# cc-ai/climategan

Hardware: AMD Instinct MI355X
Metric: 640x640 images/sec (G+D step): per-domain sample slots per second of the joint Masker+Painter training step (update_G + update_D), global batch 32 per domain (higher is better)
Workload: dtype bf16

## Files before the change

### climategan_amd/_lib.py

```python
import ctypes as C
import os
from pathlib import Path

_HERE = Path(__file__).resolve().parent
LIB_PATH = Path(os.environ["CGAN_LIB"]).resolve() if os.environ.get("CGAN_LIB") else _HERE / "libcgan_hip.so"

CGAN_F16, CGAN_BF16, CGAN_F32 = 0, 1, 2
ACT_NONE, ACT_RELU, ACT_LRELU, ACT_TANH, ACT_SIGMOID = 0, 1, 2, 3, 4
PAD_ZERO, PAD_REFLECT = 0, 1
ABI_VERSION = 1


class ConvDesc(C.Structure):
    _fields_ = [
        ("dtype", C.c_int32), ("n", C.c_int32), ("h_in", C.c_int32), ("w_in", C.c_int32),
        ("c_in", C.c_int32), ("c_out", C.c_int32),
        ("kh", C.c_int32), ("kw", C.c_int32), ("stride", C.c_int32), ("pad", C.c_int32), ("dilation", C.c_int32),
        ("pad_mode", C.c_int32), ("h_out", C.c_int32), ("w_out", C.c_int32), ("in_upsample", C.c_int32),
        ("act", C.c_int32), ("act_slope", C.c_float), ("has_bias", C.c_int32), ("has_residual", C.c_int32),
        ("residual_upsample", C.c_int32),
    ]


class NormStatsDesc(C.Structure):
# ... 121 lines not shown
    "cgan_spade_packed_weight_bytes": (C.c_size_t, [C.POINTER(SpadeDesc)]),
    "cgan_spade_pack_weights": (C.c_int, [_P, _P, _P, _P, _P, _P, _P, C.POINTER(SpadeDesc), _P]),
    "cgan_spade_fused_fwd": (C.c_int, [_P, _P, _P, _P, _P, _P, C.POINTER(SpadeDesc), _P]),
    "cgan_spade_fused_fwd_train": (C.c_int, [_P, _P, _P, _P, _P, _P, _P, C.POINTER(SpadeDesc), _P]),
    "cgan_spectral_norm_workspace_bytes": (C.c_size_t, [C.c_int32, C.c_int32]),
    "cgan_spectral_norm_power_iter": (C.c_int, [_P, _P, _P, _P, C.c_int32, C.c_int32, _P, C.c_size_t, _P]),
    "cgan_spectral_norm_power_iter_batched": (C.c_int, [_P, C.c_int32, C.c_int32, C.c_int32, _P]),
    "cgan_extra_adam_multi_tensor": (C.c_int, [_P, C.c_int32, C.c_int64, C.c_int32, C.c_int32, C.c_int32, C.c_double,
                                               C.c_double, C.c_double, C.c_double, C.c_double, _P]),
    "cgan_grads_nonfinite_check_multi_tensor": (C.c_int, [_P, C.c_int32, C.c_int64, C.c_double, C.c_int32, _P, _P]),
    "cgan_adam_multi_tensor": (C.c_int, [_P, C.c_int32, C.c_int64] + [C.c_double] * 6 + [_P, _P]),
    "cgan_rmsprop_multi_tensor": (C.c_int, [_P, C.c_int32, C.c_int64] + [C.c_double] * 5 + [_P, _P]),
    "cgan_amp_optim_finish": (C.c_int, [_P, C.c_int32, _P, _P]),
    "cgan_nchw_to_nhwc": (C.c_int, [_P, _P, _P, C.c_int32, C.c_int32, C.c_int32, C.c_int32, C.c_int32, C.c_int32, _P]),
    "cgan_nhwc_to_nchw": (C.c_int, [_P, _P, _P, _P, C.c_int32, C.c_int32, C.c_int32, C.c_int32, C.c_int32, C.c_int32, _P]),
    "cgan_resize_nearest_nhwc": (C.c_int, [_P, _P, C.c_int32, C.c_int32, C.c_int32, C.c_int32, C.c_int32, C.c_int32,
                                           C.c_int32, C.c_int32, C.c_int32, _P]),
    "cgan_avgpool3x3s2_nhwc": (C.c_int, [_P, _P, C.c_int32, C.c_int32, C.c_int32, C.c_int32, C.c_int32, _P]),
    "cgan_maxpool3x3s2_nhwc": (C.c_int, [_P, _P, C.c_int32, C.c_int32, C.c_int32, C.c_int32, C.c_int32, _P]),
    "cgan_resize_bilinear_nhwc": (C.c_int, [_P, _P, C.c_int32, C.c_int32, C.c_int32, C.c_int32, C.c_int32, C.c_int32,
                                            C.c_int32, C.c_int32, _P]),
    "cgan_resize_bicubic_nhwc": (C.c_int, [_P, _P, C.c_int32, C.c_int32, C.c_int32, C.c_int32, C.c_int32, C.c_int32,
                                           C.c_int32, _P]),
    "cgan_sumpool2x2_nhwc": (C.c_int, [_P, _P, C.c_int32, C.c_int32, C.c_int32, C.c_int32, C.c_int32, _P]),
    "cgan_reflect_pad_bwd_nhwc": (C.c_int, [_P, _P, C.c_int32, C.c_int32, C.c_int32, C.c_int32, C.c_int32, C.c_int32, _P]),
    "cgan_copy_channels_nhwc": (C.c_int, [_P, _P, C.c_int64, C.c_int32, C.c_int32, C.c_int32, C.c_int32, _P]),
    "cgan_eltwise_nhwc": (C.c_int, [_P, _P, _P, C.c_int32, C.c_int32, C.c_int64, _P]),
    "cgan_fold_bn": (C.c_int, [_P, _P, _P, _P, _P, _P, C.c_float, _P, _P, C.c_int32, C.c_int64, _P]),
    "cgan_act_bwd": (C.c_int, [_P, _P, _P, C.c_int32, C.c_int32, C.c_float, C.c_int64, _P]),
    "cgan_instnorm_act_bwd_workspace_bytes": (C.c_size_t, [C.POINTER(NormStatsDesc)]),
    "cgan_instnorm_act_bwd": (C.c_int, [_P, _P, _P, _P, C.POINTER(NormStatsDesc), C.c_int32, C.c_float, _P, C.c_size_t,
                                        _P]),
    "cgan_spade_bwd_prepare": (C.c_int, [_P, _P, _P, _P, _P, _P, _P, _P, _P, C.POINTER(SpadeDesc), _P]),
    "cgan_spade_hidden_bwd_workspace_bytes": (C.c_size_t, [C.POINTER(SpadeDesc)]),
    "cgan_spade_hidden_bwd": (C.c_int, [_P, _P, _P, _P, _P, _P, _P, _P, C.c_size_t, C.POINTER(SpadeDesc), _P]),
    "cgan_batchnorm_train_stats": (C.c_int, [_P, _P, _P, C.c_float, _P, _P, _P, _P, _P, _P, _P, C.POINTER(NormStatsDesc), _P,
                                             C.c_size_t, _P]),
    "cgan_batchnorm_train_stats_from_partials": (C.c_int, [_P, C.c_int32, _P, _P, C.c_float, _P, _P, _P, _P, _P, _P, _P,
                                                           C.POINTER(NormStatsDesc), _P]),
    "cgan_conv2d_stats_chunk_pixels": (C.c_int32, [C.POINTER(ConvDesc)]),
    "cgan_conv2d_nhwc_fwd_stats": (C.c_int, [_P, _P, _P, _P, _P, C.c_size_t, C.POINTER(ConvDesc), _P]),
    "cgan_bn_train_prepare": (C.c_int, [_P, _P, _P, _P, C.c_float, C.c_float, C.c_int64, _P, _P, _P, _P, _P, C.c_int32, _P]),
    "cgan_batchnorm_act_bwd_workspace_bytes": (C.c_size_t, [C.c_int32]),
    "cgan_batchnorm_act_bwd": (C.c_int, [_P, _P, _P, _P, _P, _P, _P, _P, _P, _P, _P, _P, C.c_int32, C.c_int64, C.c_int32,
                                         C.c_int32, C.c_float, _P, C.c_size_t, _P]),
    "cgan_batchnorm_act_bwd_grouped": (C.c_int, [_P, _P, _P, _P, _P, _P, _P, _P, _P, _P, _P, _P, C.c_int32, C.c_int64,
                                                 C.c_int32, C.c_int32, C.c_int32, C.c_float, _P, C.c_size_t, _P]),
    "cgan_bce_logits_nhwc": (C.c_int, [_P, C.c_int32, C.c_int64, C.c_int32, C.c_float, C.c_float, _P, _P, _P]),
    "cgan_hinge_nhwc": (C.c_int, [_P, C.c_int32, C.c_int64, C.c_int32, C.c_int32, C.c_int32, C.c_float, _P, _P, _P]),
    "cgan_l1_nhwc": (C.c_int, [_P, _P, C.c_int32, C.c_int64, C.c_float, _P, _P, _P]),
    "cgan_mse_const_nhwc": (C.c_int, [_P, C.c_int32, C.c_int64, C.c_int32, C.c_float, C.c_float, _P, _P, _P]),
    "cgan_painter_aux_losses": (C.c_int, [_P, _P, _P, C.c_int32, C.c_int32, C.c_int32, C.c_int32, C.c_float, C.c_float,
                                          C.c_float, C.c_float, _P, _P, _P]),
    "cgan_resize_bicubic_bwd_nhwc": (C.c_int, [_P, _P, C.c_int32, C.c_int32, C.c_int32, C.c_int32, C.c_int32, C.c_int32,
                                               C.c_int32, _P]),
    "cgan_spectral_norm_bwd": (C.c_int, [_P, _P, _P, _P, _P, C.c_int32, C.c_int32, _P, _P]),
    "cgan_painter_heads_fwd": (C.c_int, [_P, _P, _P, _P, _P, C.c_int32, C.c_int32, C.c_int32, C.c_int32, _P]),
    "cgan_painter_heads_bwd": (C.c_int, [_P, _P, _P, _P, C.c_int32, C.c_int32, C.c_int32, C.c_int32, _P]),
    "cgan_diffaug_fwd": (C.c_int, [_P, _P, _P, _P, C.c_int32, C.c_int32, C.c_int32, C.c_int32, C.c_int32, C.c_int32,
                                   C.c_int32, _P, _P]),
    "cgan_diffaug_bwd": (C.c_int, [_P, _P, _P, _P, C.c_int32, C.c_int32, C.c_int32, C.c_int32, C.c_int32, C.c_int32,
                                   C.c_int32, _P, _P]),
    "cgan_painter_heads_diffaug_fwd": (C.c_int, [_P, _P, _P, _P, _P, _P, _P, C.c_int32, C.c_int32, C.c_int32, C.c_int32,
                                                 C.c_int32, C.c_int32, C.c_int32, _P, _P]),
    "cgan_painter_heads_diffaug_bwd": (C.c_int, [_P, _P, _P, _P, _P, _P, C.c_int32, C.c_int32, C.c_int32, C.c_int32,
                                                 C.c_int32, C.c_int32, C.c_int32, _P, _P]),
# ... 142 lines not shown
```

### climategan_amd/autograd.py

```python
import ctypes as C

import os

import torch

from . import ops


GRAD_SCALE = 1.0


def set_grad_scale(s: float):
    global GRAD_SCALE
    GRAD_SCALE = float(s)


BN_GROUPS = 1


class bn_groups:

    def __init__(self, groups: int):
        self.groups = int(groups)

# ... 197 lines not shown
                                       pad_mode=cfg.get("pad_mode", ops.PAD_ZERO), add=add, prepacked=ctx.dgrad,
                                       relu_out=relu_out).t
        dw = db = None
        if ctx.needs_input_grad[1] or (ctx.has_bias and ctx.needs_input_grad[2]):
            dw, db = ops.conv2d_bwd_weight(
                ops.NHWC(x_t, cfg["c_in"]), dy, tuple(weight.shape), stride=cfg["stride"], pad=cfg["pad"],
                dilation=cfg["dilation"], want_bias=ctx.has_bias, pad_mode=cfg.get("pad_mode", ops.PAD_ZERO))
        return dx_t, dw, db, None, None


class InstNormActFn(torch.autograd.Function):

    @staticmethod
    def forward(ctx, x_t, c, eps, act, slope):
        x = ops.NHWC(x_t, c)
        mean, rstd = ops.instnorm_stats(x, eps=eps)
        out = ops.norm_act_apply(x, mean, rstd, act=act, slope=slope)
        ctx.c, ctx.act, ctx.slope = c, act, slope
        ctx.save_for_backward(out.t, rstd)
        return out.t

    @staticmethod
    def backward(ctx, dy_t):
        out_t, rstd = ctx.saved_tensors
        dx = ops.instnorm_act_bwd(ops.NHWC(out_t, ctx.c), ops.NHWC(dy_t.contiguous(), ctx.c), rstd, act=ctx.act,
                                  slope=ctx.slope)
        return dx.t, None, None, None, None


_SPADE_REMAT_GAMMA = os.environ.get("CGAN_SPADE_REMAT_GAMMA") == "1"


_SPADE_FUSED_BWD = os.environ.get("CGAN_SPADE_FUSED_BWD", "1") != "0"


class SpadeFn(torch.autograd.Function):

    @staticmethod
    def forward(ctx, x_t, cond_t, mean, rstd, w_sh, b_sh, w_g, b_g, w_b, b_b, packed, cfg):
        x = ops.NHWC(x_t, cfg["c"])
        cond = ops.NHWC(cond_t, cfg["cond_c"])
        gamma_t = None
        if _SPADE_REMAT_GAMMA or not any(ctx.needs_input_grad):
            y = ops.spade_fused(x, mean, rstd, cond, packed, act=cfg["act"], slope=cfg["slope"],
                                x_upsample=cfg["x_upsample"])
        else:
            y, gamma = ops.spade_fused(x, mean, rstd, cond, packed, act=cfg["act"], slope=cfg["slope"],
                                       x_upsample=cfg["x_upsample"], want_gamma=True)
            gamma_t = gamma.t
        ctx.cfg = cfg
        ctx.save_for_backward(x_t, cond_t, mean, rstd, y.t, w_sh, b_sh, w_g, b_g, w_b, b_b, gamma_t)
        return y.t

    @staticmethod
    def backward(ctx, dy_t):
        cfg = ctx.cfg
        x_t, cond_t, mean, rstd, y_t, w_sh, b_sh, w_g, b_g, w_b, b_b, gamma_t = ctx.saved_tensors
        c, dt = cfg["c"], y_t.dtype
        x, y = ops.NHWC(x_t, c), ops.NHWC(y_t, c)
        dy = ops.NHWC(dy_t.contiguous(), c)
        h, w = y.h, y.w
        seg = ops.resize_nearest(ops.NHWC(cond_t, cfg["cond_c"]), (h, w), cs_out=ops.cs8(cfg["cond_c"]))
        pw_sh = ops.pack_conv_weight(w_sh, b_sh, dt)
        actv = ops.conv2d(seg, pw_sh, pad=1, act=ops.ACT_RELU)
        gamma = ops.NHWC(gamma_t, c) if gamma_t is not None else ops.conv2d(actv, ops.pack_conv_weight(w_g, b_g, dt), pad=1)
        dgb, xhat, dxhat = ops.spade_bwd_prepare(dy, y, x, mean, rstd, gamma, act=cfg["act"], slope=cfg["slope"],
                                                 x_upsample=cfg["x_upsample"])
        del gamma
        w_gb = torch.cat([w_g.detach(), w_b.detach()], dim=0)
        want_gb, want_sh = any(ctx.needs_input_grad[6:10]), any(ctx.needs_input_grad[4:6])
        dw_gb = db_gb = dw_sh = db_sh = None
        if want_gb:
            dw_gb, db_gb = ops.conv2d_bwd_weight(actv, dgb, tuple(w_gb.shape), pad=1)
        fused = (_SPADE_FUSED_BWD and want_sh and not ctx.needs_input_grad[1] and cfg["cond_c"] <= 4 and h * w >= 6400
                 and w_sh.shape[0] == 128 and dgb.t.nbytes < ops.ABI_MAX_BYTES and seg.t.nbytes < ops.ABI_MAX_BYTES)
        d_pre = None
        if fused:
            dw_sh, db_sh = ops.spade_hidden_bwd(dgb, w_gb, seg, pw_sh, c)
        elif want_sh or ctx.needs_input_grad[1]:
            d_pre = ops.conv2d_bwd_data(dgb, w_gb, (actv.n, h, w), pad=1, relu_out=actv)
        del dgb, actv
        if want_sh and not fused:
            dw_sh, db_sh = ops.conv2d_bwd_weight(seg, d_pre, tuple(w_sh.shape), pad=1)
        dcond_t = None
        if ctx.needs_input_grad[1]:
            d_seg = ops.conv2d_bwd_data(d_pre, w_sh.detach(), (seg.n, h, w), pad=1)
            dcond_t = ops.resize_nearest_bwd(d_seg, (cond_t.shape[1], cond_t.shape[2]), cond_t.shape[3]).t
        del d_pre
        if cfg.get("batch_stats"):
            nn_, hh, ww, cs = xhat.t.shape
            dx = ops.instnorm_act_bwd(ops.NHWC(xhat.t.view(1, nn_ * hh * ww, 1, cs), c),
                                      ops.NHWC(dxhat.t.view(1, nn_ * hh * ww, 1, cs), c), rstd[0:1].contiguous(),
                                      act=ops.ACT_NONE)
            dx = ops.NHWC(dx.t.view(nn_, hh, ww, cs), c)
        else:
            dx = ops.instnorm_act_bwd(xhat, dxhat, rstd, act=ops.ACT_NONE)
        if cfg["x_upsample"]:
            dx = ops.sumpool2x2(dx)
        dx_t = dx.t if ctx.needs_input_grad[0] else None
        if not want_gb:
            return (dx_t, dcond_t, None, None, dw_sh, db_sh, None, None, None, None, None, None)
        return (dx_t, dcond_t, None, None, dw_sh, db_sh, dw_gb[:c].contiguous(), db_gb[:c].contiguous(),
                dw_gb[c:].contiguous(), db_gb[c:].contiguous(), None, None)


class MakeMCondFn(torch.autograd.Function):

    @staticmethod
    def forward(ctx, d_t, s_t, x, s_c):
        ctx.s_c, ctx.with_x = s_c, x is not None
        ctx.save_for_backward(d_t, s_t)
        return ops.make_m_cond(ops.NHWC(d_t, 1), ops.NHWC(s_t, s_c), x).t

    @staticmethod
    def backward(ctx, dcond_t):
        d_t, s_t = ctx.saved_tensors
        cond_c = 1 + ctx.s_c + (3 if ctx.with_x else 0)
        dd, ds = ops.make_m_cond_bwd(ops.NHWC(dcond_t.contiguous(), cond_c), ops.NHWC(d_t, 1), ops.NHWC(s_t, ctx.s_c),
                                     ctx.with_x)
        return dd.t, ds.t, None, None


class PainterHeadsFn(torch.autograd.Function):

    @staticmethod
    def forward(ctx, fake_t, x, m, want_d, want_vgg):
        d_in, v_in = ops.painter_heads(ops.NHWC(fake_t, 3), x, m, fake_t.dtype, want_d, want_vgg)
        ctx.save_for_backward(m)
        ctx.want = (want_d, want_vgg)
        empty = fake_t.new_empty(0)
# ... 599 lines not shown
```

### climategan_amd/csrc/train_ops.hip

```cpp
#include "cgan_common.h"

namespace {

__host__ __device__ inline int grid_for_n(long total) {
  long g = (total + 255) / 256;
  return (int)(g < 1 ? 1 : (g > 8192 ? 8192 : g));
}

__device__ __forceinline__ float act_grad_from_out(float out, int act, float slope) {
  switch (act) {
    case CGAN_ACT_RELU: return out > 0.f ? 1.f : 0.f;
    case CGAN_ACT_LRELU: return out > 0.f ? 1.f : slope;
    case CGAN_ACT_TANH: return 1.f - out * out;
    case CGAN_ACT_SIGMOID: return out * (1.f - out);
    default: return 1.f;
  }
}

template <typename T>
__global__ void act_bwd_kernel(const uint16_t* __restrict__ out, const uint16_t* dy, uint16_t* dx, int act, float slope,
                               long groups) {
  for (long i = (long)blockIdx.x * blockDim.x + threadIdx.x; i < groups; i += (long)gridDim.x * blockDim.x) {
    const u32x4 o = CGAN_LD_STREAM(reinterpret_cast<const u32x4*>(out) + i);
    const u32x4 g = CGAN_LD_STREAM(reinterpret_cast<const u32x4*>(dy) + i);
// ... 206 lines not shown
        const float xh = live ? (xv[hh] - mean[(long)n * cs + ch]) * rstd[(long)n * cs + ch] : 0.f;
        rxh[hh] = xh;
        rdx[hh] = dz * (1.f + g2[hh]);
        rdg[hh] = dz * xh;
        dbeta[2 * e + hh] = dz;
      }
      oxh[e] = pack2<T>(rxh[0], rxh[1]);
      odx[e] = pack2<T>(rdx[0], rdx[1]);
      odg[e] = pack2<T>(rdg[0], rdg[1]);
    }
    CGAN_ST_STREAM(oxh, reinterpret_cast<u32x4*>(xhat) + i);
    CGAN_ST_STREAM(odx, reinterpret_cast<u32x4*>(dxhat) + i);
    uint16_t* row = dgb + pix * cs2;
    if (cg * 8 + 8 <= c) {
      *reinterpret_cast<u32x4*>(row + cg * 8) = odg;
    } else {
#pragma unroll
      for (int e = 0; e < 8; ++e)
        if (cg * 8 + e < c) row[cg * 8 + e] = (uint16_t)((odg[e >> 1] >> ((e & 1) * 16)) & 0xffffu);
    }
    if (cg * 8 + 8 <= c && (c & 3) == 0) {
      const u32x4 obt = {pack2<T>(dbeta[0], dbeta[1]), pack2<T>(dbeta[2], dbeta[3]), pack2<T>(dbeta[4], dbeta[5]),
                         pack2<T>(dbeta[6], dbeta[7])};
      if ((c & 7) == 0) {
        *reinterpret_cast<u32x4*>(row + c + cg * 8) = obt;
      } else {
        *reinterpret_cast<u32x2*>(row + c + cg * 8) = (u32x2){obt[0], obt[1]};
        *reinterpret_cast<u32x2*>(row + c + cg * 8 + 4) = (u32x2){obt[2], obt[3]};
      }
    } else {
#pragma unroll
      for (int e = 0; e < 8; ++e)
        if (cg * 8 + e < c) row[c + cg * 8 + e] = bits_of<T>(dbeta[e]);
    }
  }
}

__global__ void bn_train_prepare_kernel(const float* __restrict__ mean, const float* __restrict__ rstd,
                                        const float* __restrict__ gamma, const float* __restrict__ beta, float eps,
                                        float momentum, float count, float* __restrict__ running_mean,
                                        float* __restrict__ running_var, float* __restrict__ mean_out,
                                        float* __restrict__ rstd_out, long long* __restrict__ num_batches_tracked, int c,
                                        int cs) {
  const int ch = blockIdx.x * blockDim.x + threadIdx.x;
  if (ch == 0 && num_batches_tracked) *num_batches_tracked += 1;
  if (ch >= cs) return;
  float m = 0.f, r = 0.f;
  if (ch < c) {
    const float mu = mean[ch], rs = rstd[ch];
    r = rs * (gamma ? gamma[ch] : 1.f);
    m = mu - ((beta && r != 0.f) ? beta[ch] / r : 0.f);
    if (running_mean) {
      const float var_b = 1.f / (rs * rs) - eps;
      const float var_u = count > 1.f ? var_b * count / (count - 1.f) : var_b;
      running_mean[ch] = (1.f - momentum) * running_mean[ch] + momentum * mu;
      running_var[ch] = (1.f - momentum) * running_var[ch] + momentum * var_u;
    }
  }
  mean_out[ch] = m;
  rstd_out[ch] = r;
}

constexpr int BN_BWD_MAX_CHUNKS = 512;
template <int MASK>
__device__ __forceinline__ float bn_bwd_act_grad(float ov, float xv, float fm, float fr, float gneg) {
  if (MASK == 0) return 1.f;
// ... 438 lines not shown
    long blocks = (d->hw + (long)rows * 4 - 1) / ((long)rows * 4);
    const long cap = 8192 / d->n > 0 ? 8192 / d->n : 1;
    blocks = blocks < 1 ? 1 : (blocks > cap ? cap : blocks);
    DISPATCH_T(d->dtype, in_bwd_apply_kernel, dim3((unsigned)blocks, d->n), dim3(256), 0, s, (const uint16_t*)out,
               (const uint16_t*)dy, rstd, (const float*)workspace, (uint16_t*)dx, d->hw, cs, d->c, act, act_slope);
  }
  CGAN_CHECK_LAUNCH("instnorm_act_bwd");
  return CGAN_OK;
}

extern "C" int cgan_spade_bwd_prepare(const void* dy, const void* y, const void* x, const float* mean, const float* rstd,
                                      const void* gamma, void* dgb, void* xhat, void* dxhat, const CganSpadeDesc* d,
                                      void* stream) {
  CGAN_REQUIRE(d && dy && y && x && mean && rstd && gamma && dgb && xhat && dxhat, "spade_bwd_prepare: null pointer");
  CGAN_REQUIRE(d->dtype == CGAN_F16 || d->dtype == CGAN_BF16, "spade_bwd_prepare: bad dtype %d", d->dtype);
  CGAN_REQUIRE(d->n > 0 && d->h > 0 && d->w > 0 && d->c > 0, "spade_bwd_prepare: bad shape");
  CGAN_REQUIRE(d->act == CGAN_ACT_NONE || d->act == CGAN_ACT_LRELU, "spade_bwd_prepare: Unsupported activation: %d", d->act);
  if (d->x_upsample) CGAN_REQUIRE((d->h % 2) == 0 && (d->w % 2) == 0, "spade_bwd_prepare: x_upsample needs even h/w");
  const int cs = cgan_cs(d->c), cs2 = cgan_cs(2 * d->c);
  const long npix = (long)d->n * d->h * d->w;
  hipStream_t s = (hipStream_t)stream;
  if (cs2 != 2 * d->c) {
    hipError_t e = hipMemsetAsync(dgb, 0, (size_t)npix * cs2 * 2, s);
    if (e != hipSuccess) {
      cgan_set_error("spade_bwd_prepare: hipMemsetAsync failed: %s", hipGetErrorString(e));
      return CGAN_ERR_HIP;
    }
  }
  const long groups = npix * (cs / 8);
  DISPATCH_T(d->dtype, spade_bwd_prepare_kernel, dim3(grid_for_n(groups)), dim3(256), 0, s, (const uint16_t*)dy,
             (const uint16_t*)y, (const uint16_t*)x, mean, rstd, (const uint16_t*)gamma, (uint16_t*)dgb, (uint16_t*)xhat,
             (uint16_t*)dxhat, d->h, d->w, d->c, cs, cs2, d->x_upsample, d->act, d->act_slope, groups);
  CGAN_CHECK_LAUNCH("spade_bwd_prepare");
  return CGAN_OK;
}

extern "C" int cgan_bn_train_prepare(const float* batch_mean, const float* batch_rstd, const float* gamma,
                                     const float* beta, float eps, float momentum, int64_t count, float* running_mean,
                                     float* running_var, float* mean_out, float* rstd_out,
                                     int64_t* num_batches_tracked, int32_t c, void* stream) {
  CGAN_REQUIRE(batch_mean && batch_rstd && mean_out && rstd_out, "bn_train_prepare: null pointer");
  CGAN_REQUIRE((running_mean == nullptr) == (running_var == nullptr), "bn_train_prepare: running stats go together");
  CGAN_REQUIRE(c > 0 && count > 0, "bn_train_prepare: bad shape");
  const int cs = cgan_cs(c);
  hipLaunchKernelGGL(bn_train_prepare_kernel, dim3((cs + 255) / 256), dim3(256), 0, (hipStream_t)stream, batch_mean,
                     batch_rstd, gamma, beta, eps, momentum, (float)count, running_mean, running_var, mean_out, rstd_out,
                     (long long*)num_batches_tracked, c, cs);
  CGAN_CHECK_LAUNCH("bn_train_prepare");
  return CGAN_OK;
}

extern "C" size_t cgan_batchnorm_act_bwd_workspace_bytes(int32_t c) {
  return c > 0 ? (size_t)cgan_cs(c) * (3 + 2 * (size_t)BN_BWD_MAX_CHUNKS) * sizeof(float) : 0;
}

extern "C" int cgan_batchnorm_act_bwd(const void* x, const void* out, const void* dy, const float* batch_mean,
                                      const float* batch_rstd, const float* gamma, const float* fold_mean,
                                      const float* fold_rstd, void* dx, float* dgamma, float* dbeta, void* dz_out,
                                      int32_t dtype, int64_t npix, int32_t c, int32_t act, float act_slope,
                                      void* workspace, size_t workspace_bytes, void* stream) {
  return cgan_batchnorm_act_bwd_grouped(x, out, dy, batch_mean, batch_rstd, gamma, fold_mean, fold_rstd, dx, dgamma, dbeta,
                                        dz_out, dtype, npix, c, 1, act, act_slope, workspace, workspace_bytes, stream);
}

extern "C" int cgan_batchnorm_act_bwd_grouped(const void* x, const void* out, const void* dy, const float* batch_mean,
                                              const float* batch_rstd, const float* gamma, const float* fold_mean,
// ... 128 lines not shown
```

### climategan_amd/ops.py

```python
import ctypes as C
import functools
import inspect
import os
from dataclasses import dataclass
from typing import Optional, Tuple

import torch

from . import _lib
from ._lib import (ACT_LRELU, ACT_NONE, ACT_RELU, ACT_SIGMOID, ACT_TANH, CGAN_BF16, CGAN_F16, PAD_REFLECT,
                   PAD_ZERO, ConvDesc, NormStatsDesc, PackItem, SnItem, SpadeDesc)

_DT = {torch.float16: CGAN_F16, torch.bfloat16: CGAN_BF16}


def touch(*tensors) -> None:
    ts = [t for t in tensors if t is not None]
    if ts:
        torch.autograd.graph.increment_version(ts)


MAX_MAP_BYTES = 2 ** 31
ABI_MAX_BYTES = 2 ** 31

# ... 1285 lines not shown
    if x.c != pk.c or cond.c != pk.cond_c:
        raise RuntimeError("spade_fused: channel mismatch (x %d vs %d, cond %d vs %d)" % (x.c, pk.c, cond.c, pk.cond_c))
    if cond.cs != cs4(cond.c):
        raise RuntimeError("spade_fused: cond must be stored with round_up(cond_c,4) channels")
    if x.t.dtype != pk.dtype or cond.t.dtype != pk.dtype:
        raise RuntimeError("spade_fused: dtype mismatch")
    h, w = (x.h * 2, x.w * 2) if x_upsample else (x.h, x.w)
    d = _spade_desc(x.dtype_id, x.n, h, w, x.c, x_upsample, cond.h, cond.w, cond.c, act, slope)
    y = _empty((x.n, h, w, x.cs), dtype=x.t.dtype, device=x.t.device)
    lib = _lib.load()
    if want_gamma:
        gamma = _empty_like(y)
        _lib.check(lib.cgan_spade_fused_fwd_train(_ptr(x.t), _ptr(mean), _ptr(rstd), _ptr(cond.t), _ptr(pk.buf), _ptr(y),
                                                  _ptr(gamma), C.byref(d), _stream()), "cgan_spade_fused_fwd_train")
        return NHWC(y, x.c), NHWC(gamma, x.c)
    _lib.check(lib.cgan_spade_fused_fwd(_ptr(x.t), _ptr(mean), _ptr(rstd), _ptr(cond.t), _ptr(pk.buf), _ptr(y),
                                        C.byref(d), _stream()), "cgan_spade_fused_fwd")
    return NHWC(y, x.c)


@_batch_chunked("dy", "y", "x", "mean", "rstd", "gamma", out_bytes_per_sample=lambda g: g("y").h * g("y").w * cs8(2 * g("y").c) * 2)
def spade_bwd_prepare(dy: NHWC, y: NHWC, x: NHWC, mean, rstd, gamma: NHWC, act=ACT_NONE, slope=0.2, x_upsample=False):
    _need_cuda(dy.t, y.t, x.t, mean, rstd, gamma.t)
    c = y.c
    d = _spade_desc(y.dtype_id, y.n, y.h, y.w, c, x_upsample, y.h, y.w, 3, act, slope)
    dgb = _empty((y.n, y.h, y.w, cs8(2 * c)), dtype=y.t.dtype, device=y.t.device)
    xhat = _empty_like(y.t)
    dxhat = _empty_like(y.t)
    lib = _lib.load()
    _lib.check(lib.cgan_spade_bwd_prepare(_ptr(dy.t), _ptr(y.t), _ptr(x.t), _ptr(mean), _ptr(rstd), _ptr(gamma.t),
                                          _ptr(dgb), _ptr(xhat), _ptr(dxhat), C.byref(d), _stream()),
               "cgan_spade_bwd_prepare")
    return NHWC(dgb, 2 * c), NHWC(xhat, c), NHWC(dxhat, c)


@_batch_chunked("x", "mean", "rstd", "gamma", "beta")
def pair_spade_apply(x: "PairMap", mean, rstd, gamma: "PairMap", beta: "PairMap", act=ACT_NONE, slope=0.2,
                     x_upsample=False) -> "PairMap":
    _need_cuda(x.t, mean, rstd, gamma.t, beta.t)
    h, w = (x.h * 2, x.w * 2) if x_upsample else (x.h, x.w)
    if (gamma.n, gamma.h, gamma.w, gamma.c) != (x.n, h, w, x.c) or gamma.t.shape != beta.t.shape or gamma.t.dtype != x.t.dtype:
        raise RuntimeError("pair_spade_apply: gamma / beta must be pair maps of x's channels at the output extent")
    y = _empty((x.n, h, w, x.nb * x.cs), dtype=x.t.dtype, device=x.t.device)
    _lib.check(_lib.load().cgan_pair_spade_apply(_ptr(x.t), _ptr(mean), _ptr(rstd), _ptr(gamma.t), _ptr(beta.t), _ptr(y), x.dtype_id,
                                                 x.n, h, w, x.c, int(bool(x_upsample)), int(act), float(slope), _stream()),
               "cgan_pair_spade_apply")
    return PairMap(y, x.c)


def spade_hidden_bwd(dgb: NHWC, w_gb: torch.Tensor, seg: NHWC, pw_shared: PackedConv, c: int, want_bias=True):
    _need_cuda(dgb.t, w_gb, seg.t)
    n, h, w = dgb.n, dgb.h, dgb.w
    hidden = w_gb.shape[1]
    if seg.c > 4 or hidden != 128 or (seg.n, seg.h, seg.w) != (n, h, w) or dgb.c != 2 * c or w_gb.shape[0] != 2 * c:
        raise RuntimeError("spade_hidden_bwd: needs a <= 4-channel conditioning image at the map's extent and hidden width 128")
    lib = _lib.load()
    w_gb = w_gb.detach().contiguous().float()
    dconv = _conv_desc(dgb.dtype_id, n, h, w, hidden, 2 * c, 3, 3, 1, 1, 1, PAD_ZERO, has_bias=False)
    nbytes = lib.cgan_conv2d_dgrad_packed_weight_bytes(C.byref(dconv))
    if nbytes == 0:
        _lib.check(-1, "cgan_conv2d_dgrad_packed_weight_bytes")
    packed = _empty(nbytes, dtype=torch.uint8, device=w_gb.device)
    _lib.check(lib.cgan_conv2d_pack_weight_dgrad(_ptr(w_gb), _ptr(None), _ptr(packed), C.byref(dconv), _stream()),
               "cgan_conv2d_pack_weight_dgrad")
    d = _spade_desc(dgb.dtype_id, n, h, w, c, False, h, w, seg.c, ACT_NONE)
    ws = _empty(lib.cgan_spade_hidden_bwd_workspace_bytes(C.byref(d)), dtype=torch.uint8, device=dgb.t.device)
# ... 493 lines not shown
```

### include/climategan_hip.h

```cpp
#ifndef CLIMATEGAN_HIP_H
#define CLIMATEGAN_HIP_H

#include <stddef.h>
#include <stdint.h>

#ifdef __cplusplus
extern "C" {
#endif

#define CGAN_ABI_VERSION 1

typedef enum {
  CGAN_OK = 0,
  CGAN_ERR_BAD_ARG = -1,
  CGAN_ERR_UNSUPPORTED = -2,
  CGAN_ERR_WORKSPACE = -3,
  CGAN_ERR_HIP = -4
} cgan_status_t;

typedef enum { CGAN_F16 = 0, CGAN_BF16 = 1, CGAN_F32 = 2  } cgan_dtype_t;
typedef enum { CGAN_ACT_NONE = 0, CGAN_ACT_RELU = 1, CGAN_ACT_LRELU = 2, CGAN_ACT_TANH = 3, CGAN_ACT_SIGMOID = 4 } cgan_act_t;
typedef enum { CGAN_PAD_ZERO = 0, CGAN_PAD_REFLECT = 1 } cgan_pad_t;

static inline int cgan_cs(int c) { return (c + 7) & ~7; }
// ... 137 lines not shown

int cgan_nchw_to_nhwc(const float* x, const float* mask, void* y, int32_t dtype, int32_t n, int32_t c, int32_t h,
                      int32_t w, int32_t cs, void* stream);
int cgan_nhwc_to_nchw(const void* y, const float* paste_x, const float* paste_m, float* out, int32_t dtype,
                      int32_t n, int32_t c, int32_t h, int32_t w, int32_t cs, void* stream);
int cgan_resize_nearest_nhwc(const void* x, void* y, int32_t dtype, int32_t n, int32_t c, int32_t h_in, int32_t w_in,
                             int32_t cs_in, int32_t h_out, int32_t w_out, int32_t cs_out, void* stream);
int cgan_avgpool3x3s2_nhwc(const void* x, void* y, int32_t dtype, int32_t n, int32_t c, int32_t h_in, int32_t w_in,
                           void* stream);

int cgan_maxpool3x3s2_nhwc(const void* x, void* y, int32_t dtype, int32_t n, int32_t c, int32_t h_in, int32_t w_in,
                           void* stream);
int cgan_resize_bilinear_nhwc(const void* x, void* y, int32_t dtype, int32_t n, int32_t c, int32_t h_in, int32_t w_in,
                              int32_t h_out, int32_t w_out, int32_t align_corners, void* stream);
int cgan_resize_bicubic_nhwc(const void* x, void* y, int32_t dtype, int32_t n, int32_t c, int32_t h_in, int32_t w_in,
                             int32_t h_out, int32_t w_out, void* stream);
int cgan_sumpool2x2_nhwc(const void* x, void* y, int32_t dtype, int32_t n, int32_t c, int32_t h_out, int32_t w_out,
                         void* stream);
int cgan_reflect_pad_bwd_nhwc(const void* dx_padded, void* dx, int32_t dtype, int32_t n, int32_t c, int32_t h, int32_t w,
                              int32_t pad, void* stream);
int cgan_copy_channels_nhwc(const void* src, void* dst, int64_t npix, int32_t c, int32_t cs_src, int32_t cs_dst,
                            int32_t c_off, void* stream);
int cgan_eltwise_nhwc(const void* a, const void* b, void* y, int32_t dtype, int32_t op, int64_t numel, void* stream);
int cgan_fold_bn(const float* w, const float* bias, const float* gamma, const float* beta, const float* mean,
                 const float* var, float eps, float* w_out, float* b_out, int32_t c_out, int64_t per_out, void* stream);

int cgan_act_bwd(const void* out, const void* dy, void* dx, int32_t dtype, int32_t act, float act_slope,
                 int64_t numel, void* stream);
size_t cgan_instnorm_act_bwd_workspace_bytes(const CganNormStatsDesc* d);
int cgan_instnorm_act_bwd(const void* out, const void* dy, const float* rstd, void* dx, const CganNormStatsDesc* d,
                          int32_t act, float act_slope, void* workspace, size_t workspace_bytes, void* stream);
int cgan_spade_bwd_prepare(const void* dy, const void* y, const void* x, const float* mean, const float* rstd,
                           const void* gamma, void* dgb, void* xhat, void* dxhat, const CganSpadeDesc* d, void* stream);
size_t cgan_spade_hidden_bwd_workspace_bytes(const CganSpadeDesc* d);
int cgan_spade_hidden_bwd(const void* dgb, const void* packed_dgrad_gb, const void* cond_hw, const void* packed_w_shared,
                          const float* bias_shared_padded, float* dw_shared, float* db_shared, void* workspace,
                          size_t workspace_bytes, const CganSpadeDesc* d, void* stream);
int cgan_bn_train_prepare(const float* batch_mean, const float* batch_rstd, const float* gamma, const float* beta,
                          float eps, float momentum, int64_t count, float* running_mean, float* running_var,
                          float* mean_out, float* rstd_out, int64_t* num_batches_tracked, int32_t c, void* stream);
int cgan_batchnorm_train_stats(const void* x, const float* gamma, const float* beta, float momentum, float* running_mean,
                               float* running_var, int64_t* num_batches_tracked, float* batch_mean, float* batch_rstd,
                               float* mean_out, float* rstd_out, const CganNormStatsDesc* d, void* workspace,
                               size_t workspace_bytes, void* stream);
int cgan_batchnorm_train_stats_from_partials(float* partial, int32_t chunk_pixels, const float* gamma,
                                             const float* beta, float momentum, float* running_mean, float* running_var,
                                             int64_t* num_batches_tracked, float* batch_mean, float* batch_rstd,
                                             float* mean_out, float* rstd_out, const CganNormStatsDesc* d, void* stream);
size_t cgan_batchnorm_act_bwd_workspace_bytes(int32_t c);
int cgan_batchnorm_act_bwd(const void* x, const void* out, const void* dy, const float* batch_mean,
                           const float* batch_rstd, const float* gamma, const float* fold_mean, const float* fold_rstd,
                           void* dx, float* dgamma, float* dbeta, void* dz_out, int32_t dtype, int64_t npix, int32_t c,
                           int32_t act, float act_slope, void* workspace, size_t workspace_bytes, void* stream);
int cgan_batchnorm_act_bwd_grouped(const void* x, const void* out, const void* dy, const float* batch_mean,
                                   const float* batch_rstd, const float* gamma, const float* fold_mean,
                                   const float* fold_rstd, void* dx, float* dgamma, float* dbeta, void* dz_out,
                                   int32_t dtype, int64_t npix_total, int32_t c, int32_t groups, int32_t act,
                                   float act_slope, void* workspace, size_t workspace_bytes, void* stream);
int cgan_bce_logits_nhwc(const void* x, int32_t dtype, int64_t npix, int32_t c, float target, float weight,
                         float* loss_accum, void* dx, void* stream);
int cgan_hinge_nhwc(const void* x, int32_t dtype, int64_t npix, int32_t c, int32_t target_is_real,
                    int32_t for_discriminator, float weight, float* loss_accum, void* dx, void* stream);
int cgan_mse_const_nhwc(const void* x, int32_t dtype, int64_t npix, int32_t c, float target, float weight, float* loss_accum,
                        void* dx, void* stream);
int cgan_painter_aux_losses(const void* fake_nhwc, const float* x_nchw, const float* m_nchw, int32_t dtype, int32_t n,
                            int32_t h, int32_t w, float w_tv_h, float w_tv_w, float w_context, float w_reconstruction,
// ... 249 lines not shown
```

Baseline: 57.79.

## Fuse SPADE backward elementwise prep with instnorm reduction and upsample sumpool

Replaces the SPADE backward prepare, instance-norm backward and 2x2 sumpool sequence with two kernels. The first produces dgb and dxhat while accumulating per-channel instance-norm reduction partials, and no longer materializes xhat. The second recomputes xhat from x and applies the norm gradient with the upsample folded in, writing dx at input resolution. This cuts full-resolution memory traffic and kernel launches, at the cost of more complex kernels. The batch_stats path still uses the old route.

```diff
diff --git a/climategan_amd/_lib.py b/climategan_amd/_lib.py
--- a/climategan_amd/_lib.py
+++ b/climategan_amd/_lib.py
@@ -177,6 +177,9 @@
     "cgan_instnorm_act_bwd": (C.c_int, [_P, _P, _P, _P, C.POINTER(NormStatsDesc), C.c_int32, C.c_float, _P, C.c_size_t,
                                         _P]),
     "cgan_spade_bwd_prepare": (C.c_int, [_P, _P, _P, _P, _P, _P, _P, _P, _P, C.POINTER(SpadeDesc), _P]),
+    "cgan_spade_bwd_stage_workspace_bytes": (C.c_size_t, [C.POINTER(SpadeDesc)]),
+    "cgan_spade_bwd_stage": (C.c_int, [_P, _P, _P, _P, _P, _P, _P, _P, _P, C.c_size_t, C.POINTER(SpadeDesc), _P]),
+    "cgan_spade_bwd_apply": (C.c_int, [_P, _P, _P, _P, _P, _P, C.POINTER(SpadeDesc), _P]),
     "cgan_spade_hidden_bwd_workspace_bytes": (C.c_size_t, [C.POINTER(SpadeDesc)]),
     "cgan_spade_hidden_bwd": (C.c_int, [_P, _P, _P, _P, _P, _P, _P, _P, C.c_size_t, C.POINTER(SpadeDesc), _P]),
     "cgan_batchnorm_train_stats": (C.c_int, [_P, _P, _P, C.c_float, _P, _P, _P, _P, _P, _P, _P, C.POINTER(NormStatsDesc), _P,
diff --git a/climategan_amd/autograd.py b/climategan_amd/autograd.py
--- a/climategan_amd/autograd.py
+++ b/climategan_amd/autograd.py
@@ -253,6 +253,7 @@
 
 
 _SPADE_FUSED_BWD = os.environ.get("CGAN_SPADE_FUSED_BWD", "1") != "0"
+_SPADE_FUSED_ELT = os.environ.get("CGAN_SPADE_FUSED_ELT", "1") != "0"
 
 
 class SpadeFn(torch.autograd.Function):
@@ -285,8 +286,13 @@
         pw_sh = ops.pack_conv_weight(w_sh, b_sh, dt)
         actv = ops.conv2d(seg, pw_sh, pad=1, act=ops.ACT_RELU)
         gamma = ops.NHWC(gamma_t, c) if gamma_t is not None else ops.conv2d(actv, ops.pack_conv_weight(w_g, b_g, dt), pad=1)
-        dgb, xhat, dxhat = ops.spade_bwd_prepare(dy, y, x, mean, rstd, gamma, act=cfg["act"], slope=cfg["slope"],
-                                                 x_upsample=cfg["x_upsample"])
+        fused_elt = _SPADE_FUSED_ELT and not cfg.get("batch_stats")
+        if fused_elt:
+            dgb, dxhat, sums = ops.spade_bwd_stage(dy, y, x, mean, rstd, gamma, act=cfg["act"], slope=cfg["slope"],
+                                                   x_upsample=cfg["x_upsample"])
+        else:
+            dgb, xhat, dxhat = ops.spade_bwd_prepare(dy, y, x, mean, rstd, gamma, act=cfg["act"], slope=cfg["slope"],
+                                                     x_upsample=cfg["x_upsample"])
         del gamma
         w_gb = torch.cat([w_g.detach(), w_b.detach()], dim=0)
         want_gb, want_sh = any(ctx.needs_input_grad[6:10]), any(ctx.needs_input_grad[4:6])
@@ -308,7 +314,9 @@
             d_seg = ops.conv2d_bwd_data(d_pre, w_sh.detach(), (seg.n, h, w), pad=1)
             dcond_t = ops.resize_nearest_bwd(d_seg, (cond_t.shape[1], cond_t.shape[2]), cond_t.shape[3]).t
         del d_pre
-        if cfg.get("batch_stats"):
+        if fused_elt:
+            dx = ops.spade_bwd_apply(dxhat, x, mean, rstd, sums, x_upsample=cfg["x_upsample"])
+        elif cfg.get("batch_stats"):
             nn_, hh, ww, cs = xhat.t.shape
             dx = ops.instnorm_act_bwd(ops.NHWC(xhat.t.view(1, nn_ * hh * ww, 1, cs), c),
                                       ops.NHWC(dxhat.t.view(1, nn_ * hh * ww, 1, cs), c), rstd[0:1].contiguous(),
@@ -316,7 +324,7 @@
             dx = ops.NHWC(dx.t.view(nn_, hh, ww, cs), c)
         else:
             dx = ops.instnorm_act_bwd(xhat, dxhat, rstd, act=ops.ACT_NONE)
-        if cfg["x_upsample"]:
+        if cfg["x_upsample"] and not fused_elt:
             dx = ops.sumpool2x2(dx)
         dx_t = dx.t if ctx.needs_input_grad[0] else None
         if not want_gb:
diff --git a/climategan_amd/csrc/train_ops.hip b/climategan_amd/csrc/train_ops.hip
--- a/climategan_amd/csrc/train_ops.hip
+++ b/climategan_amd/csrc/train_ops.hip
@@ -262,6 +262,195 @@
 #pragma unroll
       for (int e = 0; e < 8; ++e)
         if (cg * 8 + e < c) row[c + cg * 8 + e] = bits_of<T>(dbeta[e]);
+    }
+  }
+}
+
+template <typename T, int UPS>
+__global__ __launch_bounds__(256) void spade_bwd_stage_kernel(
+    const uint16_t* __restrict__ dy, const uint16_t* __restrict__ y, const uint16_t* __restrict__ x,
+    const float* __restrict__ mean, const float* __restrict__ rstd, const uint16_t* __restrict__ gamma,
+    uint16_t* __restrict__ dgb, uint16_t* __restrict__ dxhat, float* __restrict__ partial, int h, int w, int c, int cs,
+    int cs2, int ppb, int act, float slope) {
+  extern __shared__ __attribute__((aligned(16))) float sm[];
+  const int hw = h * w;
+  const int cg_total = cs / 8;
+  const int cgb = cg_total < 256 ? cg_total : 256;
+  const int PL = 256 / cgb;
+  const int n = blockIdx.z, cg0 = blockIdx.y * cgb;
+  const int p0 = blockIdx.x * ppb, p1 = min(hw, p0 + ppb);
+  const int t = threadIdx.x, cgl = t % cgb, pl = t / cgb;
+  const int cg = cg0 + cgl;
+  float s1[8], s2[8];
+#pragma unroll
+  for (int e = 0; e < 8; ++e) s1[e] = s2[e] = 0.f;
+  if (pl < PL && cg < cg_total) {
+    float mu[8], rs[8];
+#pragma unroll
+    for (int e = 0; e < 8; ++e) {
+      mu[e] = mean[(size_t)n * cs + cg * 8 + e];
+      rs[e] = rstd[(size_t)n * cs + cg * 8 + e];
+    }
+    const size_t base = (size_t)n * hw * cs + cg * 8;
+    const size_t xbase = UPS ? (size_t)n * (hw >> 2) * cs + cg * 8 : base;
+    const int w2 = w >> 1;
+#pragma unroll 2
+    for (int p = p0 + pl; p < p1; p += PL) {
+      const size_t off = base + (size_t)p * cs;
+      size_t xoff = off;
+      if (UPS) {
+        const unsigned oy = (unsigned)p / (unsigned)w, ox = (unsigned)p - oy * (unsigned)w;
+        xoff = xbase + ((size_t)(oy >> 1) * w2 + (ox >> 1)) * cs;
+      }
+      const u32x4 vdy = CGAN_LD_STREAM(reinterpret_cast<const u32x4*>(dy + off));
+      const u32x4 vy = CGAN_LD_STREAM(reinterpret_cast<const u32x4*>(y + off));
+      const u32x4 vg = CGAN_LD_STREAM(reinterpret_cast<const u32x4*>(gamma + off));
+      const u32x4 vx = *reinterpret_cast<const u32x4*>(x + xoff);
+      u32x4 odx, odg;
+      float dbeta[8];
+#pragma unroll
+      for (int e = 0; e < 4; ++e) {
+        float a[2], b[2], g2[2], xv[2], rxh[2], rdx[2], rdg[2];
+        unpack2<T>(vdy[e], a[0], a[1]);
+        unpack2<T>(vy[e], b[0], b[1]);
+        unpack2<T>(vg[e], g2[0], g2[1]);
+        unpack2<T>(vx[e], xv[0], xv[1]);
+#pragma unroll
+        for (int hh = 0; hh < 2; ++hh) {
+          const int k = 2 * e + hh;
+          const bool live = cg * 8 + k < c;
+          const float dz = live ? a[hh] * act_grad_from_out(b[hh], act, slope) : 0.f;
+          const float xh = live ? (xv[hh] - mu[k]) * rs[k] : 0.f;
+          rxh[hh] = xh;
+          rdx[hh] = dz * (1.f + g2[hh]);
+          rdg[hh] = dz * xh;
+          dbeta[k] = dz;
+        }
+        odx[e] = pack2<T>(rdx[0], rdx[1]);
+        odg[e] = pack2<T>(rdg[0], rdg[1]);
+        float q0, q1;
+        unpack2<T>(odx[e], q0, q1);
+        s1[2 * e] += q0; s2[2 * e] += q0 * rxh[0];
+        s1[2 * e + 1] += q1; s2[2 * e + 1] += q1 * rxh[1];
+      }
+      CGAN_ST_STREAM(odx, reinterpret_cast<u32x4*>(dxhat + off));
+      uint16_t* row = dgb + ((size_t)n * hw + p) * cs2;
+      if (cg * 8 + 8 <= c) {
+        *reinterpret_cast<u32x4*>(row + cg * 8) = odg;
+      } else {
+#pragma unroll
+        for (int e = 0; e < 8; ++e)
+          if (cg * 8 + e < c) row[cg * 8 + e] = (uint16_t)((odg[e >> 1] >> ((e & 1) * 16)) & 0xffffu);
+      }
+      if (cg * 8 + 8 <= c && (c & 3) == 0) {
+        const u32x4 obt = {pack2<T>(dbeta[0], dbeta[1]), pack2<T>(dbeta[2], dbeta[3]), pack2<T>(dbeta[4], dbeta[5]),
+                           pack2<T>(dbeta[6], dbeta[7])};
+        if ((c & 7) == 0) {
+          *reinterpret_cast<u32x4*>(row + c + cg * 8) = obt;
+        } else {
+          *reinterpret_cast<u32x2*>(row + c + cg * 8) = (u32x2){obt[0], obt[1]};
+          *reinterpret_cast<u32x2*>(row + c + cg * 8 + 4) = (u32x2){obt[2], obt[3]};
+        }
+      } else {
+#pragma unroll
+        for (int e = 0; e < 8; ++e)
+          if (cg * 8 + e < c) row[c + cg * 8 + e] = bits_of<T>(dbeta[e]);
+      }
+    }
+  }
+  if (pl < PL) {
+#pragma unroll
+    for (int e = 0; e < 8; ++e) {
+      sm[((pl * cgb + cgl) * 8 + e) * 2] = s1[e];
+      sm[((pl * cgb + cgl) * 8 + e) * 2 + 1] = s2[e];
+    }
+  }
+  __syncthreads();
+  for (int ch = t; ch < cgb * 8; ch += 256) {
+    if (cg0 * 8 + ch >= cs) continue;
+    float a = 0.f, b = 0.f;
+    for (int l = 0; l < PL; ++l) {
+      a += sm[((l * cgb) * 8 + ch) * 2];
+      b += sm[((l * cgb) * 8 + ch) * 2 + 1];
+    }
+    float* o = partial + (((size_t)n * gridDim.x + blockIdx.x) * cs + cg0 * 8 + ch) * 2;
+    o[0] = a;
+    o[1] = b;
+  }
+}
+
+template <typename T, int UPS>
+__global__ __launch_bounds__(256) void spade_bwd_apply_kernel(const uint16_t* __restrict__ dxhat,
+                                                              const uint16_t* __restrict__ x,
+                                                              const float* __restrict__ mean,
+                                                              const float* __restrict__ rstd,
+                                                              const float* __restrict__ sums, uint16_t* __restrict__ dx,
+                                                              int h, int w, int cs, int c) {
+  const int cg_total = cs / 8;
+  const int tpp = cg_total < 256 ? cg_total : 256;
+  const int rows = 256 / tpp;
+  const int cgl = threadIdx.x % tpp, prow = threadIdx.x / tpp;
+  if (prow >= rows) return;
+  const int n = blockIdx.y;
+  const int hw = h * w;
+  const int opix = UPS ? hw >> 2 : hw;
+  const int w2 = w >> 1;
+  const float inv_hw = 1.f / (float)hw;
+  dxhat += (size_t)n * hw * cs;
+  x += (size_t)n * opix * cs;
+  dx += (size_t)n * opix * cs;
+  for (int cg = cgl; cg < cg_total; cg += tpp) {
+    float mu[8], rs[8], m1[8], m2[8];
+#pragma unroll
+    for (int e = 0; e < 8; ++e) {
+      const int ch = cg * 8 + e;
+      const float* sp = sums + ((size_t)n * cs + ch) * 2;
+      mu[e] = mean[(size_t)n * cs + ch];
+      rs[e] = rstd[(size_t)n * cs + ch];
+      m1[e] = sp[0] * inv_hw * (UPS ? 4.f : 1.f);
+      m2[e] = sp[1] * inv_hw * (UPS ? 4.f : 1.f);
+    }
+#pragma unroll 2
+    for (int p = blockIdx.x * rows + prow; p < opix; p += gridDim.x * rows) {
+      const size_t off = (size_t)p * cs + cg * 8;
+      const u32x4 vx = CGAN_LD_STREAM(reinterpret_cast<const u32x4*>(x + off));
+      u32x4 d0, d1, d2, d3;
+      if (UPS) {
+        const unsigned ly = (unsigned)p / (unsigned)w2, lx = (unsigned)p - ly * (unsigned)w2;
+        const size_t q = ((size_t)(2 * ly) * w + 2 * lx) * cs + cg * 8;
+        d0 = CGAN_LD_STREAM(reinterpret_cast<const u32x4*>(dxhat + q));
+        d1 = CGAN_LD_STREAM(reinterpret_cast<const u32x4*>(dxhat + q + cs));
+        d2 = CGAN_LD_STREAM(reinterpret_cast<const u32x4*>(dxhat + q + (size_t)w * cs));
+        d3 = CGAN_LD_STREAM(reinterpret_cast<const u32x4*>(dxhat + q + (size_t)w * cs + cs));
+      } else {
+        d0 = CGAN_LD_STREAM(reinterpret_cast<const u32x4*>(dxhat + off));
+        d1 = d2 = d3 = d0;
+      }
+      u32x4 r;
+#pragma unroll
+      for (int e = 0; e < 4; ++e) {
+        float xv[2], g[2], res[2];
+        unpack2<T>(vx[e], xv[0], xv[1]);
+        unpack2<T>(d0[e], g[0], g[1]);
+        if (UPS) {
+          float t0, t1;
+          unpack2<T>(d1[e], t0, t1);
+          g[0] += t0; g[1] += t1;
+          unpack2<T>(d2[e], t0, t1);
+          g[0] += t0; g[1] += t1;
+          unpack2<T>(d3[e], t0, t1);
+          g[0] += t0; g[1] += t1;
+        }
+#pragma unroll
+        for (int hh = 0; hh < 2; ++hh) {
+          const int k = 2 * e + hh;
+          const float xh = (xv[hh] - mu[k]) * rs[k];
+          const float v = rs[k] * (g[hh] - m1[k] - xh * m2[k]);
+          res[hh] = cg * 8 + k < c ? v : 0.f;
+        }
+        r[e] = pack2<T>(res[0], res[1]);
+      }
+      CGAN_ST_STREAM(r, reinterpret_cast<u32x4*>(dx + off));
     }
   }
 }
@@ -766,6 +955,93 @@
              (const uint16_t*)y, (const uint16_t*)x, mean, rstd, (const uint16_t*)gamma, (uint16_t*)dgb, (uint16_t*)xhat,
              (uint16_t*)dxhat, d->h, d->w, d->c, cs, cs2, d->x_upsample, d->act, d->act_slope, groups);
   CGAN_CHECK_LAUNCH("spade_bwd_prepare");
+  return CGAN_OK;
+}
+
+static bool spade_bwd_map_fits(const CganSpadeDesc* d) {
+  return (size_t)d->n * d->h * d->w * cgan_cs(d->c) * 2 < ((size_t)1 << 31);
+}
+
+static CganNormStatsDesc spade_bwd_norm_desc(const CganSpadeDesc* d) {
+  CganNormStatsDesc nd = {};
+  nd.dtype = d->dtype;
+  nd.n = d->n;
+  nd.hw = d->h * d->w;
+  nd.c = d->c;
+  return nd;
+}
+
+extern "C" size_t cgan_spade_bwd_stage_workspace_bytes(const CganSpadeDesc* d) {
+  if (!d || d->n <= 0 || d->c <= 0 || d->h <= 0 || d->w <= 0 || !spade_bwd_map_fits(d)) return 0;
+  const CganNormStatsDesc nd = spade_bwd_norm_desc(d);
+  return cgan_instnorm_act_bwd_workspace_bytes(&nd);
+}
+
+extern "C" int cgan_spade_bwd_stage(const void* dy, const void* y, const void* x, const float* mean, const float* rstd,
+                                    const void* gamma, void* dgb, void* dxhat, void* workspace, size_t workspace_bytes,
+                                    const CganSpadeDesc* d, void* stream) {
+  CGAN_REQUIRE(d && dy && y && x && mean && rstd && gamma && dgb && dxhat && workspace, "spade_bwd_stage: null pointer");
+  CGAN_REQUIRE(d->dtype == CGAN_F16 || d->dtype == CGAN_BF16, "spade_bwd_stage: bad dtype %d", d->dtype);
+  CGAN_REQUIRE(d->n > 0 && d->h > 0 && d->w > 0 && d->c > 0, "spade_bwd_stage: bad shape");
+  CGAN_REQUIRE(d->n <= 65535, "spade_bwd_stage: at most 65535 samples per call");
+  CGAN_REQUIRE(d->act == CGAN_ACT_NONE || d->act == CGAN_ACT_LRELU, "spade_bwd_stage: Unsupported activation: %d", d->act);
+  if (d->x_upsample) CGAN_REQUIRE((d->h % 2) == 0 && (d->w % 2) == 0, "spade_bwd_stage: x_upsample needs even h/w");
+  CGAN_REQUIRE(spade_bwd_map_fits(d), "spade_bwd_stage: a 16-bit map of 2 GiB or more (only dgb may be that large)");
+  CGAN_REQUIRE(workspace_bytes >= cgan_spade_bwd_stage_workspace_bytes(d), "spade_bwd_stage: workspace too small");
+  const int cs = cgan_cs(d->c), cs2 = cgan_cs(2 * d->c), cg_total = cs / 8;
+  const size_t npix = (size_t)d->n * d->h * d->w;
+  hipStream_t s = (hipStream_t)stream;
+  if (cs2 != 2 * d->c) {
+    hipError_t e = hipMemsetAsync(dgb, 0, npix * cs2 * 2, s);
+    if (e != hipSuccess) {
+      cgan_set_error("spade_bwd_stage: hipMemsetAsync failed: %s", hipGetErrorString(e));
+      return CGAN_ERR_HIP;
+    }
+  }
+  const CganNormStatsDesc nd = spade_bwd_norm_desc(d);
+  int cgb, PL, ppb, chunks;
+  in_bwd_plan(&nd, cgb, PL, ppb, chunks);
+  float* sums = (float*)workspace;
+  float* partial = sums + (size_t)d->n * cs * 2;
+  const size_t smem = (size_t)PL * cgb * 8 * 2 * sizeof(float);
+  const dim3 grid(chunks, ceil_div(cg_total, cgb), d->n);
+  if (d->x_upsample)
+    DISPATCH_T2(d->dtype, spade_bwd_stage_kernel, 1, grid, dim3(256), smem, s, (const uint16_t*)dy, (const uint16_t*)y,
+                (const uint16_t*)x, mean, rstd, (const uint16_t*)gamma, (uint16_t*)dgb, (uint16_t*)dxhat, partial, d->h,
+                d->w, d->c, cs, cs2, ppb, d->act, d->act_slope);
+  else
+    DISPATCH_T2(d->dtype, spade_bwd_stage_kernel, 0, grid, dim3(256), smem, s, (const uint16_t*)dy, (const uint16_t*)y,
+                (const uint16_t*)x, mean, rstd, (const uint16_t*)gamma, (uint16_t*)dgb, (uint16_t*)dxhat, partial, d->h,
+                d->w, d->c, cs, cs2, ppb, d->act, d->act_slope);
+  hipLaunchKernelGGL(in_bwd_finalize_kernel, dim3(d->n * cs / 8), dim3(256), 0, s, (const float*)partial, sums, d->n, cs,
+                     chunks);
+  CGAN_CHECK_LAUNCH("spade_bwd_stage");
+  return CGAN_OK;
+}
+
+extern "C" int cgan_spade_bwd_apply(const void* dxhat, const void* x, const float* mean, const float* rstd,
+                                    const float* sums, void* dx, const CganSpadeDesc* d, void* stream) {
+  CGAN_REQUIRE(d && dxhat && x && mean && rstd && sums && dx, "spade_bwd_apply: null pointer");
+  CGAN_REQUIRE(d->dtype == CGAN_F16 || d->dtype == CGAN_BF16, "spade_bwd_apply: bad dtype %d", d->dtype);
+  CGAN_REQUIRE(d->n > 0 && d->h > 0 && d->w > 0 && d->c > 0, "spade_bwd_apply: bad shape");
+  CGAN_REQUIRE(d->n <= 65535, "spade_bwd_apply: at most 65535 samples per call");
+  if (d->x_upsample) CGAN_REQUIRE((d->h % 2) == 0 && (d->w % 2) == 0, "spade_bwd_apply: x_upsample needs even h/w");
+  CGAN_REQUIRE(spade_bwd_map_fits(d), "spade_bwd_apply: a 16-bit map of 2 GiB or more");
+  const int cs = cgan_cs(d->c), cg_total = cs / 8;
+  const int tpp = cg_total < 256 ? cg_total : 256, rows = 256 / tpp;
+  const long opix = (long)d->h * d->w / (d->x_upsample ? 4 : 1);
+  const long per_thread = d->x_upsample ? 2 : 4;
+  long blocks = (opix + rows * per_thread - 1) / (rows * per_thread);
+  const long cap = 8192 / d->n > 0 ? 8192 / d->n : 1;
+  blocks = blocks < 1 ? 1 : (blocks > cap ? cap : blocks);
+  hipStream_t s = (hipStream_t)stream;
+  if (d->x_upsample)
+    DISPATCH_T2(d->dtype, spade_bwd_apply_kernel, 1, dim3((unsigned)blocks, d->n), dim3(256), 0, s,
+                (const uint16_t*)dxhat, (const uint16_t*)x, mean, rstd, sums, (uint16_t*)dx, d->h, d->w, cs, d->c);
+  else
+    DISPATCH_T2(d->dtype, spade_bwd_apply_kernel, 0, dim3((unsigned)blocks, d->n), dim3(256), 0, s,
+                (const uint16_t*)dxhat, (const uint16_t*)x, mean, rstd, sums, (uint16_t*)dx, d->h, d->w, cs, d->c);
+  CGAN_CHECK_LAUNCH("spade_bwd_apply");
   return CGAN_OK;
 }
 
diff --git a/climategan_amd/ops.py b/climategan_amd/ops.py
--- a/climategan_amd/ops.py
+++ b/climategan_amd/ops.py
@@ -1341,6 +1341,38 @@
                                           _ptr(dgb), _ptr(xhat), _ptr(dxhat), C.byref(d), _stream()),
                "cgan_spade_bwd_prepare")
     return NHWC(dgb, 2 * c), NHWC(xhat, c), NHWC(dxhat, c)
+
+
+@_batch_chunked("dy", "y", "x", "mean", "rstd", "gamma")
+def spade_bwd_stage(dy: NHWC, y: NHWC, x: NHWC, mean, rstd, gamma: NHWC, act=ACT_NONE, slope=0.2, x_upsample=False):
+    _need_cuda(dy.t, y.t, x.t, mean, rstd, gamma.t)
+    c = y.c
+    d = _spade_desc(y.dtype_id, y.n, y.h, y.w, c, x_upsample, y.h, y.w, 3, act, slope)
+    lib = _lib.load()
+    nbytes = lib.cgan_spade_bwd_stage_workspace_bytes(C.byref(d))
+    if nbytes == 0:
+        _lib.check(-1, "cgan_spade_bwd_stage_workspace_bytes")
+    ws = _empty(nbytes, dtype=torch.uint8, device=y.t.device)
+    dgb = _empty((y.n, y.h, y.w, cs8(2 * c)), dtype=y.t.dtype, device=y.t.device)
+    dxhat = _empty_like(y.t)
+    _lib.check(lib.cgan_spade_bwd_stage(_ptr(dy.t), _ptr(y.t), _ptr(x.t), _ptr(mean), _ptr(rstd), _ptr(gamma.t),
+                                        C.c_void_p(dgb.data_ptr()), _ptr(dxhat), _ptr(ws), nbytes, C.byref(d), _stream()),
+               "cgan_spade_bwd_stage")
+    sums = ws[:y.n * y.cs * 8].view(torch.float32).view(y.n, y.cs, 2)
+    return NHWC(dgb, 2 * c), NHWC(dxhat, c), sums
+
+
+@_batch_chunked("dxhat", "x", "mean", "rstd", "sums")
+def spade_bwd_apply(dxhat: NHWC, x: NHWC, mean, rstd, sums, x_upsample=False) -> NHWC:
+    _need_cuda(dxhat.t, x.t, mean, rstd, sums)
+    k = 2 if x_upsample else 1
+    if (x.n, x.h * k, x.w * k, x.cs) != (dxhat.n, dxhat.h, dxhat.w, dxhat.cs) or not x.t.is_contiguous():
+        raise RuntimeError("spade_bwd_apply: x %s does not match dxhat %s" % (tuple(x.t.shape), tuple(dxhat.t.shape)))
+    d = _spade_desc(dxhat.dtype_id, dxhat.n, dxhat.h, dxhat.w, dxhat.c, x_upsample, dxhat.h, dxhat.w, 3, ACT_NONE)
+    dx = _empty_like(x.t)
+    _lib.check(_lib.load().cgan_spade_bwd_apply(_ptr(dxhat.t), _ptr(x.t), _ptr(mean), _ptr(rstd), _ptr(sums), _ptr(dx),
+                                                C.byref(d), _stream()), "cgan_spade_bwd_apply")
+    return NHWC(dx, dxhat.c)
 
 
 @_batch_chunked("x", "mean", "rstd", "gamma", "beta")
diff --git a/include/climategan_hip.h b/include/climategan_hip.h
--- a/include/climategan_hip.h
+++ b/include/climategan_hip.h
@@ -193,6 +193,12 @@
                           int32_t act, float act_slope, void* workspace, size_t workspace_bytes, void* stream);
 int cgan_spade_bwd_prepare(const void* dy, const void* y, const void* x, const float* mean, const float* rstd,
                            const void* gamma, void* dgb, void* xhat, void* dxhat, const CganSpadeDesc* d, void* stream);
+size_t cgan_spade_bwd_stage_workspace_bytes(const CganSpadeDesc* d);
+int cgan_spade_bwd_stage(const void* dy, const void* y, const void* x, const float* mean, const float* rstd,
+                         const void* gamma, void* dgb, void* dxhat, void* workspace, size_t workspace_bytes,
+                         const CganSpadeDesc* d, void* stream);
+int cgan_spade_bwd_apply(const void* dxhat, const void* x, const float* mean, const float* rstd, const float* sums,
+                         void* dx, const CganSpadeDesc* d, void* stream);
 size_t cgan_spade_hidden_bwd_workspace_bytes(const CganSpadeDesc* d);
 int cgan_spade_hidden_bwd(const void* dgb, const void* packed_dgrad_gb, const void* cond_hw, const void* packed_w_shared,
                           const float* bias_shared_padded, float* dw_shared, float* db_shared, void* workspace,
```

After: 58.44, median of 4. 1.01x the previous value.
